# Rocco9999/2048_Q-Learning

Measured on AMD Instinct MI355X. Metric: env_steps_per_sec, higher is better.
Workload: dtype u8

## Files before the change

2048_q-learning_amd/csrc/q2048_core.hpp:

```cpp
#pragma once
#include <stdint.h>
#include <math.h>

#if defined(__HIPCC__)
#define Q_HD __host__ __device__ __forceinline__
#else
#define Q_HD inline
#endif

#include "q2048_luts.inc"

namespace q2048 {

constexpr uint32_t kStreamStep = 0u, kStreamReset = 1u, kStreamOver = 2u;

struct Draws { uint32_t x0, x1, x2, x3; };

#ifndef Q2048_PHILOX_ROUNDS
#define Q2048_PHILOX_ROUNDS 10
#endif
Q_HD Draws philox4x32_10(uint32_t c0, uint32_t c1, uint32_t c2, uint32_t c3, uint32_t k0,
                         uint32_t k1) {
#pragma unroll
  for (int r = 0; r < Q2048_PHILOX_ROUNDS; ++r) {
    const uint64_t p0 = (uint64_t)0xD2511F53u * c0;
    const uint64_t p1 = (uint64_t)0xCD9E8D57u * c2;
    const uint32_t n0 = (uint32_t)(p1 >> 32) ^ c1 ^ k0;
    const uint32_t n2 = (uint32_t)(p0 >> 32) ^ c3 ^ k1;
    c1 = (uint32_t)p1;
    c3 = (uint32_t)p0;
    c0 = n0;
    c2 = n2;
    k0 += 0x9E3779B9u;
    k1 += 0xBB67AE85u;
  }
  return Draws{c0, c1, c2, c3};
}

Q_HD Draws draws(uint64_t seed, uint64_t env_id, uint32_t ctr, uint32_t stream) {
  return philox4x32_10((uint32_t)env_id, (uint32_t)(env_id >> 32), ctr, stream, (uint32_t)seed,
                       (uint32_t)(seed >> 32));
}

Q_HD double draw_uniform(uint32_t x) { return (double)x * (1.0 / 4294967296.0); }
Q_HD int draw_action(uint32_t x) { return (int)(x >> 30); }
Q_HD uint32_t draw_index(uint32_t x, uint32_t n) { return (uint32_t)(((uint64_t)x * n) >> 32); }
Q_HD bool draw_is_four(uint32_t x) { return x >= 3865470567u; }

Q_HD uint32_t nz80(uint32_t x) { return (x + 0x7f7f7f7fu) & 0x80808080u; }
Q_HD uint32_t z80(uint32_t x) { return ~(x + 0x7f7f7f7fu) & 0x80808080u; }
Q_HD uint32_t fill80(uint32_t m) { return (m << 1) - (m >> 7); }
Q_HD uint32_t fill7f(uint32_t m) { return m - (m >> 7); }
Q_HD uint32_t bsel(uint32_t m, uint32_t a, uint32_t b) { return (a & m) | (b & ~m); }

struct Board { uint32_t r0, r1, r2, r3; };

Q_HD bool operator==(const Board& a, const Board& b) {
  return ((a.r0 ^ b.r0) | (a.r1 ^ b.r1) | (a.r2 ^ b.r2) | (a.r3 ^ b.r3)) == 0;
}
Q_HD void clear(Board& b) { b = Board{0u, 0u, 0u, 0u}; }

Q_HD Board transpose(const Board& b) {
  const uint32_t a0 = (b.r0 & 0x00ff00ffu) | ((b.r1 & 0x00ff00ffu) << 8);
  const uint32_t a1 = ((b.r0 >> 8) & 0x00ff00ffu) | (b.r1 & 0xff00ff00u);
  const uint32_t b0 = (b.r2 & 0x00ff00ffu) | ((b.r3 & 0x00ff00ffu) << 8);
  const uint32_t b1 = ((b.r2 >> 8) & 0x00ff00ffu) | (b.r3 & 0xff00ff00u);
  return Board{(a0 & 0xffffu) | (b0 << 16), (a1 & 0xffffu) | (b1 << 16),
               (a0 >> 16) | (b0 & 0xffff0000u), (a1 >> 16) | (b1 & 0xffff0000u)};
}

Q_HD uint32_t pow2_sum(uint32_t v) {
  return (((1u << (v & 0xffu)) & ~1u) + ((1u << ((v >> 8) & 0xffu)) & ~1u)) +
         (((1u << ((v >> 16) & 0xffu)) & ~1u) + ((1u << (v >> 24)) & ~1u));
}

Q_HD uint32_t slide_lines(uint32_t& c0, uint32_t& c1, uint32_t& c2, uint32_t& c3) {
  uint32_t z;
#pragma unroll
  for (int rep = 0; rep < 3; ++rep) {
    z = fill7f(z80(c0));
    c0 = bsel(z, c1, c0); c1 = bsel(z, c2, c1); c2 = bsel(z, c3, c2); c3 &= ~z;
  }
#pragma unroll
  for (int rep = 0; rep < 2; ++rep) {
    z = fill7f(z80(c1));
    c1 = bsel(z, c2, c1); c2 = bsel(z, c3, c2); c3 &= ~z;
  }
  z = fill7f(z80(c2));
  c2 = bsel(z, c3, c2); c3 &= ~z;
  uint32_t e = z80(c0 ^ c1) & nz80(c0);
  uint32_t m = fill7f(e);
  c0 += e >> 7;
  const uint32_t s_a = c0 & m;
  c1 = bsel(m, c2, c1); c2 = bsel(m, c3, c2); c3 &= ~m;
// ... 43 lines not shown
  c = popc(mask & 0x3u);  ge = k >= c; k -= ge ? c : 0u; pos += ge ? 2u : 0u; mask >>= ge ? 2u : 0u;
  c = mask & 1u;          ge = k >= c; pos += ge ? 1u : 0u;
  return pos;
}

Q_HD void put_cell(Board& b, uint32_t pos, uint32_t v) {
  const uint32_t w = v << ((pos & 3u) * 8u), row = pos >> 2;
  b.r0 |= row == 0u ? w : 0u; b.r1 |= row == 1u ? w : 0u;
  b.r2 |= row == 2u ? w : 0u; b.r3 |= row == 3u ? w : 0u;
}

Q_HD void spawn(Board& b, uint32_t draw_pos, uint32_t draw_val) {
  const uint32_t em = empty_mask(b), n = popc(em);
  if (n == 0u) return;
  put_cell(b, kth_set_bit16(em, draw_index(draw_pos, n)), draw_is_four(draw_val) ? 2u : 1u);
}

Q_HD bool game_over(const Board& b) {
  const uint32_t empties = z80(b.r0) | z80(b.r1) | z80(b.r2) | z80(b.r3);
  const uint32_t vert = z80(b.r0 ^ b.r1) | z80(b.r1 ^ b.r2) | z80(b.r2 ^ b.r3);
  const uint32_t horz = (z80(b.r0 ^ (b.r0 >> 8)) | z80(b.r1 ^ (b.r1 >> 8)) |
                         z80(b.r2 ^ (b.r2 >> 8)) | z80(b.r3 ^ (b.r3 >> 8))) & 0x00808080u;
  return (empties | vert | horz) == 0u;
}

Q_HD uint32_t bytemax(uint32_t a, uint32_t b) {
  const uint32_t m = fill7f(((a | 0x80808080u) - b) & 0x80808080u);
  return bsel(m, a, b);
}
Q_HD uint32_t max_log2(const Board& b) {
  uint32_t x = bytemax(bytemax(b.r0, b.r1), bytemax(b.r2, b.r3));
  x = bytemax(x, x >> 16);
  x = bytemax(x, x >> 8);
  return x & 0xffu;
}

struct Aux {
  int32_t score;
  float ep_return;
  uint8_t prev_max;
  uint8_t cons_action;
  uint16_t cons_count;
  uint32_t episode;
};
constexpr uint8_t kNoAction = 0xFFu;
constexpr uint32_t kConsCountSat = 60000u;

Q_HD Aux aux_init() { return Aux{0, 0.0f, 1, kNoAction, 0, 0u}; }

Q_HD double lut_pow12(uint32_t L) { constexpr double t[32] = Q2048_POW12; return t[L & 31u]; }
Q_HD double lut_log2p1(uint32_t L) { constexpr double t[32] = Q2048_LOG2P1; return t[L & 31u]; }
Q_HD double lut_stall(uint32_t k) { constexpr double t[32] = Q2048_STALL; return t[k < 31u ? k : 31u]; }

Q_HD uint64_t f64_bits(double d) { union { double d; uint64_t u; } c; c.d = d; return c.u; }
Q_HD double bits_f64(uint64_t u) { union { double d; uint64_t u; } c; c.u = u; return c.d; }

Q_HD double log2_ge1(double x) {
  constexpr double inv[64] = Q2048_LOG2_INV;
  constexpr double lg[64] = Q2048_LOG2_LG;
  constexpr double a[6] = Q2048_LOG2_COEF;
  const uint64_t u = f64_bits(x);
  const int e = (int)(u >> 52) - 1023;
  const uint32_t j = (uint32_t)(u >> 46) & 63u;
  const double m = bits_f64((u & 0x000FFFFFFFFFFFFFull) | 0x3FF0000000000000ull);
  const double r = fma(m, inv[j], -1.0);
  double p = fma(r, a[5], a[4]);
  p = fma(r, p, a[3]);
  p = fma(r, p, a[2]);
  p = fma(r, p, a[1]);
  p = fma(r, p, a[0]);
  return fma(r, p, (double)e + lg[j]);
}

Q_HD double normalize_reward(double r) {
  const double v = fmin(log2_ge1(fabs(r) + 1.0), 10.0);
  return r >= 0 ? v : -v;
}

Q_HD double calculate_reward(uint32_t score, bool valid, bool over, uint32_t L, uint8_t& prev) {
  L = L < 1u ? 1u : L;
  const double cl = (double)L;
  double bonus = 0.0, r;
  if (L > prev) {
    bonus = (cl - (double)prev) * lut_pow12(L);
    prev = (uint8_t)L;
  }
  if (!valid) {
    if (over) {
      if (L >= 9u && L <= 11u) r = bonus + lut_pow12(L);
      else r = 0.0 - lut_log2p1(L);
    } else {
      r = 0.0 - 0.1 * cl;
    }
  } else {
    r = (double)score;
    if (bonus > 0) r += bonus;
    else r += cl * 0.05;
    if (L >= 9u) r += lut_pow12(L) * 2;
  }
  return normalize_reward(r);
}

struct StepOut {
  float reward;
  double reward64;
  uint32_t score;
  uint8_t done, max_log2, valid;
};

template <class BoardT>
Q_HD bool spawn_then_over(BoardT& b, bool valid, uint32_t x_pos, uint32_t x_val) {
  if (valid) spawn(b, x_pos, x_val);
  return game_over(b);
}

template <class BoardT>
Q_HD StepOut env_step(BoardT& b, Aux& a, int action, uint32_t x_pos, uint32_t x_val) {
  StepOut o;
  uint32_t score;
  const bool valid = move(b, action, score);
  const bool over = spawn_then_over(b, valid, x_pos, x_val);
  const uint32_t mx = max_log2(b);
  a.score += (int32_t)score;
  double r = calculate_reward(score, valid, over, mx, a.prev_max);
  uint32_t cnt = a.cons_count;
  if ((uint8_t)action == a.cons_action) {
    cnt = cnt + 1u < kConsCountSat ? cnt + 1u : kConsCountSat;
  } else {
    a.cons_action = (uint8_t)action;
    cnt = 1u;
  }
  a.cons_count = (uint16_t)cnt;
  bool done = !valid && over;
  if (cnt > 10u) {
    if (cnt > 100u) done = true;
    r += lut_stall(cnt - 10u);
  }
  o.reward64 = r;
  o.reward = (float)r;
  a.ep_return += o.reward;
  o.score = score;
  o.done = done;
  o.max_log2 = (uint8_t)mx;
  o.valid = valid;
  return o;
}

constexpr int kEnvDqn = 1, kEnvResetShaping = 2, kEnvPlayOnly = 4;

template <class BoardT>
Q_HD StepOut env_step_dqn(BoardT& b, Aux& a, int action, uint32_t x_pos, uint32_t x_val,
                          uint32_t y_pos, uint32_t y_val) {
  StepOut o;
  const BoardT pre = b;
  uint32_t score;
  const bool valid = move(b, action, score);
  if (valid) spawn(b, x_pos, x_val);
  bool over = false;
  if (empty_mask(pre) == 0u) {
    over = true;
    for (int act = 0; act < 4 && over; ++act) {
      BoardT t = pre;
      uint32_t s2;
      if (move(t, act, s2)) {
        spawn(t, y_pos, y_val);
        b = t;
        over = false;
      }
    }
    if (over) b = pre;
  }
  const uint32_t mx = max_log2(b);
  a.score += (int32_t)score;
  const double r = (!valid && !over) ? -10.0 : (double)score;
  o.reward64 = r;
  o.reward = (float)r;
  a.ep_return += o.reward;
  o.score = score;
  o.done = over;
  o.max_log2 = (uint8_t)mx;
  o.valid = valid;
  return o;
}

template <int ENV, class BoardT>
Q_HD StepOut env_step_profile(BoardT& b, Aux& a, int action, uint32_t x_pos, uint32_t x_val,
                              uint32_t y_pos, uint32_t y_val) {
  if constexpr ((ENV & kEnvDqn) != 0) return env_step_dqn(b, a, action, x_pos, x_val, y_pos, y_val);
  else return env_step(b, a, action, x_pos, x_val);
}

template <class BoardT>
Q_HD void reset_board(BoardT& b, Aux& a, const Draws& d) {
  clear(b);
  spawn(b, d.x0, d.x1);
  spawn(b, d.x2, d.x3);
  a.score = 0;
  a.ep_return = 0.0f;
}

template <class BoardT>
Q_HD void init_env(BoardT& b, Aux& a, uint64_t seed, uint64_t env_id) {
  a = aux_init();
  reset_board(b, a, draws(seed, env_id, 0u, kStreamReset));
}
template <class BoardT>
Q_HD void begin_episode(BoardT& b, Aux& a, uint64_t seed, uint64_t env_id,
                        bool reset_shaping = false) {
  a.episode += 1u;
  reset_board(b, a, draws(seed, env_id, a.episode, kStreamReset));
  if (reset_shaping) {
    a.prev_max = 1;
    a.cons_action = kNoAction;
    a.cons_count = 0;
  }
}

struct Words4 { uint32_t w0, w1, w2, w3; };
Q_HD uint32_t f32_bits(float f) { union { float f; uint32_t u; } c; c.f = f; return c.u; }
Q_HD float bits_f32(uint32_t u) { union { float f; uint32_t u; } c; c.u = u; return c.f; }
Q_HD Words4 aux_to_words(const Aux& a) {
  return Words4{(uint32_t)a.score, f32_bits(a.ep_return),
                (uint32_t)a.prev_max | ((uint32_t)a.cons_action << 8) | ((uint32_t)a.cons_count << 16),
                a.episode};
}
Q_HD Aux words_to_aux(const Words4& w) {
  return Aux{(int32_t)w.w0, bits_f32(w.w1), (uint8_t)(w.w2 & 0xffu), (uint8_t)((w.w2 >> 8) & 0xffu),
             (uint16_t)(w.w2 >> 16), w.w3};
}

Q_HD uint32_t pack_row(uint32_t x) {
  x &= 0x0f0f0f0fu;
  x = (x | (x >> 4)) & 0x00ff00ffu;
  return (x | (x >> 8)) & 0xffffu;
}
Q_HD uint64_t pack_key(const Board& b, bool& overflow) {
  overflow = ((b.r0 | b.r1 | b.r2 | b.r3) & 0xf0f0f0f0u) != 0u;
  return (uint64_t)(pack_row(b.r0) | (pack_row(b.r1) << 16)) |
         ((uint64_t)(pack_row(b.r2) | (pack_row(b.r3) << 16)) << 32);
}
Q_HD uint32_t unpack_row(uint32_t k) {
  k &= 0xffffu;
  k = (k | (k << 8)) & 0x00ff00ffu;
  return (k | (k << 4)) & 0x0f0f0f0fu;
}
Q_HD Board unpack_key(uint64_t key) {
  return Board{unpack_row((uint32_t)key), unpack_row((uint32_t)(key >> 16)),
               unpack_row((uint32_t)(key >> 32)), unpack_row((uint32_t)(key >> 48))};
}

Q_HD uint64_t mix64(uint64_t h) {
  h *= 0x9E3779B97F4A7C15ull;
  h ^= h >> 29;
  h *= 0xBF58476D1CE4E5B9ull;
  h ^= h >> 32;
  return h;
}
Q_HD uint64_t lane_salt(uint64_t env_id) { return mix64(env_id + 0x2048ull) | 1ull; }

Q_HD uint64_t summary_fp(uint64_t hash) { return ((hash >> 48) & 0xffffull) | 1ull; }
struct SummaryHits { uint32_t ev, empty; };
Q_HD SummaryHits summary_decode(uint64_t word, uint64_t fp, uint32_t off) {
  uint32_t e = 0u, m = 0u;
#pragma unroll
  for (uint32_t r = 0; r < 4u; ++r) {
    const uint64_t f = (word >> (16u * r)) & 0xffffull;
    e |= (uint32_t)(f == 0ull) << r;
    m |= (uint32_t)(f == fp) << r;
  }
  return SummaryHits{(((e | m) | ((e | m) << 4)) >> (off & 3u)) & 15u, e};
}
Q_HD bool summary_pop(SummaryHits& h, uint32_t off, uint32_t& r, bool& absent) {
  if (h.ev == 0u) return false;
  r = (off + (uint32_t)__builtin_ctz(h.ev)) & 3u;
  absent = ((h.empty >> r) & 1u) != 0u;
  h.ev &= h.ev - 1u;
  return true;
}

Q_HD int argmax4(float q0, float q1, float q2, float q3) {
  int b = 0;
  float m = q0;
  if (q1 > m) { m = q1; b = 1; }
  if (q2 > m) { m = q2; b = 2; }
  if (q3 > m) { m = q3; b = 3; }
  return b;
}
Q_HD float max4(float q0, float q1, float q2, float q3) { return fmaxf(fmaxf(q0, q1), fmaxf(q2, q3)); }

Q_HD int eps_greedy(double eps, uint32_t x_eps, uint32_t x_act, float q0, float q1, float q2,
                    float q3, bool& explored) {
  explored = draw_uniform(x_eps) < eps;
  return explored ? draw_action(x_act) : argmax4(q0, q1, q2, q3);
}

#if defined(__clang__)
#define Q2048_NO_CONTRACT _Pragma("clang fp contract(off)")
#else
#define Q2048_NO_CONTRACT
#endif
Q_HD double td_target(float reward, float max_q_next, bool done, double gamma) {
  Q2048_NO_CONTRACT
  const double bootstrap = gamma * (double)max_q_next;
  return (double)reward + bootstrap * (done ? 0.0 : 1.0);
}
Q_HD double td_fold(double q, double target, double lr) {
  Q2048_NO_CONTRACT
  const double step = lr * (target - q);
  return q + step;
}
Q_HD float td_value(float q_sa, float reward, float max_q_next, bool done, double lr,
                    double gamma) {
  return (float)td_fold((double)q_sa, td_target(reward, max_q_next, done, gamma), lr);
}

constexpr uint32_t kRtIdx = 65536u;
Q_HD float rt_sum(float e0, float e1, float e2, float e3) { return (e0 + e1) + (e2 + e3); }
Q_HD float rt_delta(float q_sa, float reward, float max_next, bool done, double lr, double gamma) {
  const double target = (double)reward + (gamma * (double)max_next * (done ? 0.0 : 1.0));
  return (float)((lr * 0.25) * (target - (double)q_sa));
}

}
```

2048_q-learning_amd/csrc/q2048_host.cpp:

```cpp
#include <algorithm>
#include <chrono>
#include <cstddef>
#include <cstdint>
#include <cstdlib>
#include <cstring>
#include <thread>
#include <unordered_map>
#include <vector>

#include "q2048.h"
#include "q2048_core5.hpp"

namespace {
using namespace q2048;
using u64 = unsigned long long;

constexpr uint32_t kMaxProbe = 1u << 14, kRolloutProbe = 1u << 10;
constexpr int kMaxCas = 16;
constexpr int kMaxAwait = 1 << 20;

static_assert(sizeof(q2048_aux) == 16 && sizeof(q2048_slot) == 32 && sizeof(q2048_episode) == 48, "ABI layout");
static_assert(sizeof(Aux) == sizeof(q2048_aux), "core/ABI aux mismatch");

template <int N> struct Geo;
// ... 217 lines not shown
  std::vector<std::thread> th;
  th.reserve((size_t)T);
  for (int t = 0; t < T; ++t) {
    const int64_t lo = B * t / T, hi = B * (t + 1) / T;
    th.emplace_back([=] { f(lo, hi, t); });
  }
  for (auto& x : th) x.join();
  return T;
}

struct Stats {
  uint64_t i[Q2048_NSTAT_I] = {};
  double f[Q2048_NSTAT_F] = {};
  void episode(const Aux& a, uint32_t max_l2) {
    i[Q2048_ST_SCORE] += (uint64_t)(int64_t)a.score;
    i[Q2048_ST_HIST0 + (max_l2 > 22u ? 22u : max_l2)] += 1;
    const double ret = (double)a.ep_return;
    f[Q2048_SF_RETURN] += ret;
    f[Q2048_SF_RETURN_SQ] += ret * ret;
  }
};
void stats_merge(const std::vector<Stats>& parts, int used, int64_t* gi, double* gf) {
  for (int t = 0; t < used; ++t) {
    if (gi != nullptr) for (int k = 0; k < Q2048_NSTAT_I; ++k) gi[k] += (int64_t)parts[(size_t)t].i[k];
    if (gf != nullptr) for (int k = 0; k < Q2048_NSTAT_F; ++k) gf[k] += parts[(size_t)t].f[k];
  }
}

inline bool aligned16(const void* p) { return (reinterpret_cast<uintptr_t>(p) & 15u) == 0; }
inline int check_batch(int64_t B, int n) {
  if (n != 4 && n != 5) return Q2048_ERR_UNSUPPORTED;
  if (B < 0 || B > (int64_t)0x7fffffff * 256) return Q2048_ERR_SIZE;
  return Q2048_OK;
}
inline int check_table(const void* table, int cap_log2) {
  if (table == nullptr) return Q2048_ERR_NULL;
  if (cap_log2 < 4 || cap_log2 > 40) return Q2048_ERR_SIZE;
  if (!aligned16(table)) return Q2048_ERR_ALIGN;
  return Q2048_OK;
}
constexpr uint32_t kAbiFlags = Q2048_FLAG_INDEPENDENT | Q2048_FLAG_SINGLE_ENV | Q2048_FLAG_TD_CAS | Q2048_FLAG_ENV_DQN |
                               Q2048_FLAG_RESET_SHAPING | Q2048_FLAG_PLAY_ONLY | Q2048_FLAG_NO_LEARN |
                               Q2048_FLAG_NO_NEW_ROWS | Q2048_FLAG_LINE_SUMMARY;
inline int check_flags(uint32_t flags, uint32_t refused = 0u) {
  return ((flags & ~kAbiFlags) || (flags & refused)) ? Q2048_ERR_FLAGS : Q2048_OK;
}
inline int env_bits(uint32_t flags) {
  return ((flags & Q2048_FLAG_ENV_DQN) ? kEnvDqn : 0) | ((flags & Q2048_FLAG_RESET_SHAPING) ? kEnvResetShaping : 0);
}
template <class BoardT>
inline StepOut env_step_any(int env, BoardT& b, Aux& a, int act, uint32_t x_pos, uint32_t x_val, uint32_t y_pos, uint32_t y_val) {
  return (env & kEnvDqn) ? env_step_profile<kEnvDqn>(b, a, act, x_pos, x_val, y_pos, y_val)
                         : env_step_profile<0>(b, a, act, x_pos, x_val, y_pos, y_val);
}

template <int N>
void env_init_impl(uint8_t* boards, q2048_aux* aux, int64_t B, uint64_t seed, uint64_t env_id0) {
  parallel_ranges(B, [=](int64_t lo, int64_t hi, int) {
    for (int64_t i = lo; i < hi; ++i) {
      typename Geo<N>::BoardT b;
      Aux a;
      init_env(b, a, seed, env_id0 + (uint64_t)i);
      store_board(boards, i, b);
      st_aux(aux, i, a);
    }
  });
}
template <int N>
void env_reset_impl(uint8_t* boards, q2048_aux* aux, const uint8_t* mask, int64_t B, uint64_t seed, uint64_t env_id0,
                    uint32_t flags) {
  parallel_ranges(B, [=](int64_t lo, int64_t hi, int) {
    for (int64_t i = lo; i < hi; ++i) {
      if (mask != nullptr && mask[i] == 0) continue;
      typename Geo<N>::BoardT b;
      load_board(boards, i, b);
      Aux a = ld_aux(aux, i);
      begin_episode(b, a, seed, env_id0 + (uint64_t)i, (flags & Q2048_FLAG_RESET_SHAPING) != 0);
      store_board(boards, i, b);
      st_aux(aux, i, a);
    }
  });
}
template <int N>
void env_step_impl_n(const uint8_t* boards_in, uint8_t* boards, q2048_aux* aux, const uint8_t* actions, int64_t B,
                     uint64_t seed, uint64_t env_id0, uint32_t ctr, uint32_t flags, float* reward, uint8_t* done,
                     uint8_t* max_l2, int32_t* max_tile, uint32_t* status, const uint32_t* draw_pos,
                     const uint32_t* draw_val, const uint32_t* draw_opos, const uint32_t* draw_oval, int stride) {
  const int env = env_bits(flags);
  parallel_ranges(B, [=](int64_t lo, int64_t hi, int) {
    for (int64_t i = lo; i < hi; ++i) {
      typename Geo<N>::BoardT b;
      load_board(boards_in, i, b);
      const int act = actions[i];
      if (act > 3) {
        status_or(status, Q2048_STATUS_BAD_ACTION);
        reward[i] = 0.f; done[i] = 0; max_l2[i] = 0;
        if (max_tile != nullptr) max_tile[i] = 0;
        if (boards != boards_in) store_board(boards, i, b);
        continue;
      }
      Aux a = ld_aux(aux, i);
      Draws x{0u, 0u, 0u, 0u}, y{0u, 0u, 0u, 0u};
      if (draw_pos != nullptr) {
        x.x2 = draw_pos[i * stride]; x.x3 = draw_val[i * stride];
        if (env & kEnvDqn) { y.x0 = draw_opos[i * stride]; y.x1 = draw_oval[i * stride]; }
      } else {
// ... 93 lines not shown
      const auto key_n = state_key(b_n, salt, status);
      Row rs, rn;
      bool ins_s = false, ins_n = false;
      const int64_t slot = find_or_create(table, mask, key_s, rs, ins_s, create);
      if (slot < 0 && !create) visit_get<N>(cache, i, table, mask, key_s, rs);
      rn = rs;
      const bool same = key_eq(key_n, key_s);
      int64_t slot_n = slot;
      if (!same) slot_n = find_or_create(table, mask, key_n, rn, ins_n, create);
      st.i[Q2048_ST_INSERTS] += (uint64_t)ins_s + (uint64_t)ins_n;
      const float max_next = max4(rn.q0, rn.q1, rn.q2, rn.q3);
      if (slot >= 0) {
        td_update(&table[slot], act, row_get(rs, act), reward[i], max_next, done[i] != 0, lr, gamma, cas, tdc);
      } else {
        st.i[Q2048_ST_DROPS] += 1;
        if (create) status_or(status, Q2048_STATUS_TABLE_FULL);
        else if (same) row_set(rn, act, td_value(row_get(rs, act), reward[i], max_next, done[i] != 0, lr, gamma));
      }
      visit_put<N>(cache, i, table, mask, key_n, rn, !create && slot_n < 0);
    }
    st.i[Q2048_ST_CAS_RETRY] += tdc.retries;
    st.i[Q2048_ST_CAS_FALLBACK] += tdc.fallbacks;
  });
  stats_merge(parts, used, stats_i, nullptr);
}

template <int N>
void q_lookup_impl_n(const q2048_slot* table, u64 mask, const uint8_t* boards, int64_t B, uint64_t env_id0,
                     uint32_t flags, float* q_out, uint8_t* found, uint32_t* status) {
  parallel_ranges(B, [=](int64_t lo, int64_t hi, int) {
    for (int64_t i = lo; i < hi; ++i) {
      typename Geo<N>::BoardT b;
      load_board(boards, i, b);
      const uint64_t id = (flags & Q2048_FLAG_SINGLE_ENV) ? env_id0 : env_id0 + (uint64_t)i;
      const u64 salt = (flags & Q2048_FLAG_INDEPENDENT) ? lane_salt(id) : 0ull;
      Row r;
      const int64_t slot = probe_find(table, mask, state_key(b, salt, status), r, kMaxProbe);
      q_out[4 * i] = r.q0; q_out[4 * i + 1] = r.q1; q_out[4 * i + 2] = r.q2; q_out[4 * i + 3] = r.q3;
      if (found != nullptr) found[i] = slot >= 0;
    }
  });
}

constexpr int kGroup = 16;
template <int N>
void fused_rollout_n(uint8_t* boards, q2048_aux* aux, q2048_slot* table, u64 mask, int64_t B, int steps, double eps,
                     double lr, double gamma, uint64_t seed, uint64_t env_id0, uint32_t ctr0, uint32_t flags,
                     int64_t* stats_i, double* stats_f, uint32_t* status, q2048_episode* log, int64_t log_cap,
                     uint64_t* log_count, void* cache, const uint64_t* side) {
  using BoardT = typename Geo<N>::BoardT;
  using Key = typename Geo<N>::Key;
  struct Lane {
    BoardT b; Aux a; Key key_s, key_n; Row q; int64_t slot_s; u64 salt; uint64_t id; double reward_sum;
    StepOut o; int act; bool explored, same;
  };
  const int env = env_bits(flags);
  const bool play_only = (flags & Q2048_FLAG_PLAY_ONLY) != 0, no_learn = (flags & Q2048_FLAG_NO_LEARN) != 0;
  const bool learns = !play_only && !no_learn, frozen = (flags & Q2048_FLAG_NO_NEW_ROWS) != 0;
  const bool creates = learns && !frozen, cas = (flags & Q2048_FLAG_TD_CAS) != 0;
  const bool summary = N == 5 && learns && frozen && (flags & Q2048_FLAG_LINE_SUMMARY) != 0 && side != nullptr;
  const int T = threads_for(B);
  std::vector<Stats> parts((size_t)T);
  Stats* sp = parts.data();
  const int used = parallel_ranges(B, [=](int64_t lo, int64_t hi, int tid) {
    auto find = [=](const Key& key, Row& row) {
      return summary ? probe_find_summary(table, side, mask, key, row) : probe_find(table, mask, key, row);
    };
    Stats& st = sp[tid];
    TdCounters tdc;
    bool any_drop = false;
    Lane lane[kGroup];
    for (int64_t g0 = lo; g0 < hi; g0 += kGroup) {
      const int n = (int)(hi - g0 < kGroup ? hi - g0 : kGroup);
      for (int l = 0; l < n; ++l) {
        Lane& L = lane[l];
        const int64_t i = g0 + l;
        L.id = env_id0 + (uint64_t)i;
        L.salt = (flags & Q2048_FLAG_INDEPENDENT) ? lane_salt(L.id) : 0ull;
        load_board(boards, i, L.b);
        L.a = ld_aux(aux, i);
        L.key_s = state_key(L.b, L.salt, status);
        L.q = Row{0.f, 0.f, 0.f, 0.f};
        L.slot_s = play_only ? kNoSlot : find(L.key_s, L.q);
        if (frozen && learns && L.slot_s < 0) visit_get<N>(cache, i, table, mask, L.key_s, L.q);
        L.reward_sum = 0.0;
      }
      for (int t = 0; t < steps; ++t) {
        for (int l = 0; l < n; ++l) {
          Lane& L = lane[l];
          const Draws x = draws(seed, L.id, ctr0 + (uint32_t)t, kStreamStep);
          Draws y{0u, 0u, 0u, 0u};
          if (env & kEnvDqn) y = draws(seed, L.id, ctr0 + (uint32_t)t, kStreamOver);
          L.act = eps_greedy(eps, x.x0, x.x1, L.q.q0, L.q.q1, L.q.q2, L.q.q3, L.explored);
          L.o = env_step_any(env, L.b, L.a, L.act, x.x2, x.x3, y.x0, y.x1);
          L.key_n = state_key(L.b, L.salt, status);
          L.same = key_eq(L.key_n, L.key_s);
          if (!L.same && !play_only) __builtin_prefetch(&table[key_hash(L.key_n) & mask], 1, 1);
        }
        for (int l = 0; l < n; ++l) {
          Lane& L = lane[l];
          const StepOut& o = L.o;
          const int act = L.act;
          bool ins_s = false, ins_n = false;
          if (L.slot_s < 0 && L.slot_s != kNoSlot && creates) L.slot_s = probe_insert(table, mask, L.key_s, (u64)~L.slot_s, ins_s);
          Row qn = L.q;
          int64_t slot_n = L.slot_s;
          if (!L.same) {
            if (play_only) { qn = Row{0.f, 0.f, 0.f, 0.f}; slot_n = kNoSlot; }
            else if (creates) slot_n = find_or_create(table, mask, L.key_n, qn, ins_n);
            else slot_n = find(L.key_n, qn);
          }
          const float max_next = max4(qn.q0, qn.q1, qn.q2, qn.q3);
          const bool updated = L.slot_s >= 0;
          float nq = 0.f;
          if (updated) {
            if (no_learn) nq = td_value(row_get(L.q, act), o.reward, max_next, o.done != 0, lr, gamma);
            else nq = td_update(&table[L.slot_s], act, row_get(L.q, act), o.reward, max_next, o.done != 0, lr, gamma, cas, tdc);
          } else if (frozen && learns) {
            nq = td_value(row_get(L.q, act), o.reward, max_next, o.done != 0, lr, gamma);
          }
          st.i[Q2048_ST_VALID] += o.valid != 0;
          st.i[Q2048_ST_EXPLORE] += L.explored;
          st.i[Q2048_ST_INSERTS] += (uint64_t)ins_s + (uint64_t)ins_n;
          if (!updated && learns) { st.i[Q2048_ST_DROPS] += 1; any_drop = any_drop || !frozen; }
          L.reward_sum += (double)o.reward;
          if (o.done) {
            st.i[Q2048_ST_EPISODES] += 1;
            st.episode(L.a, o.max_log2);
            if (log != nullptr) {
              const uint64_t at = __atomic_fetch_add(log_count, (uint64_t)1, __ATOMIC_RELAXED);
              if ((int64_t)at < log_cap) {
                Row ql = L.q;
                if ((updated || (frozen && learns)) && !no_learn) row_set(ql, act, nq);
                q2048_episode rec;
                rec.env_id = L.id; rec.episode = L.a.episode; rec.action = (uint8_t)act;
                rec.max_log2 = o.max_log2; rec.steps_lo = (uint16_t)(ctr0 + (uint32_t)t);
                rec.reward = o.reward; rec.total_return = L.a.ep_return; rec.score = L.a.score;
                rec.q[0] = ql.q0; rec.q[1] = ql.q1; rec.q[2] = ql.q2; rec.q[3] = ql.q3;
                rec.reserved = 0u;
                log[at] = rec;
              }
            }
            begin_episode(L.b, L.a, seed, L.id, (env & kEnvResetShaping) != 0);
            L.key_s = state_key(L.b, L.salt, status);
            L.q = Row{0.f, 0.f, 0.f, 0.f};
            L.slot_s = play_only ? kNoSlot : find(L.key_s, L.q);
          } else if (L.same) {
// ... 675 lines not shown
```

2048_q-learning_amd/csrc/q2048_kernels.hip:

```cpp
#include <hip/hip_runtime.h>
#include <stddef.h>
#include <stdint.h>

#include <cstdio>
#include <cstdlib>
#include <cstring>
#include <ctime>
#include <condition_variable>
#include <deque>
#include <functional>
#include <map>
#include <mutex>
#include <thread>
#include <vector>

#include "q2048.h"
#include "q2048_core5.hpp"

#ifdef Q2048_EXPERIMENTS
#define Q2048_XBITS(flags, shift, mask) (((flags) >> (shift)) & (mask))
#else
#define Q2048_XBITS(flags, shift, mask) 0u
#endif

// ... 848 lines not shown
      Row rn = rs;
      int64_t slot_n = slot;
      Claim claim{0ull, 0ull, false};
      if (!same) {
        slot_n = probe_find(table, mask, key_n, rn, ins_n);
        if constexpr (!frozen) slot_n = claim_issue(table, mask, slot_n, key_n, claim, ins_n);
      }
      const float max_next = max4(rn.q0, rn.q1, rn.q2, rn.q3);
      if (slot >= 0) {
        const float nq = td_update(&table[slot], act, row_get(rs, act), rew, max_next, is_done,
                                   lr, gamma, tdc, td_mode_of(flags));
        if (same) row_set(rn, act, nq);
      } else {
        dropped = true;
        if (!frozen) atomicOr(status, Q2048_STATUS_TABLE_FULL);
        else if (same)
          row_set(rn, act, td_value(row_get(rs, act), rew, max_next, is_done, lr, gamma));
      }
      bool ins_c = false;
      slot_n = claim_resolve(table, mask, key_n, claim, slot_n, ins_c);
      ins_n = ins_n || ins_c;
      if (cache != nullptr) cache_put(cache, i, key_n, cache_tag(table, mask), rn, slot_n, frozen);
    }
    const uint32_t n_ins = wave_count(ins_n) + wave_count(ins_s), n_drop = wave_count(dropped);
    if (tdc.retries) atomicAdd(&bs.i[Q2048_ST_CAS_RETRY], (u64)tdc.retries);
    if (tdc.fallbacks) atomicAdd(&bs.i[Q2048_ST_CAS_FALLBACK], (u64)tdc.fallbacks);
    if (wave_leader()) {
      if (n_ins) atomicAdd(&bs.i[Q2048_ST_INSERTS], (u64)n_ins);
      if (n_drop) atomicAdd(&bs.i[Q2048_ST_DROPS], (u64)n_drop);
    }
  }
  stats_flush(bs, stats_i, nullptr);
}

#ifdef Q2048_FUSED_MIN_WAVES
#define Q2048_FUSED_WAVES(N) Q2048_FUSED_MIN_WAVES
#else
#define Q2048_FUSED_WAVES(N) ((N) == 4 ? 6 : 5)
#endif
constexpr int kModeLearn = 0, kModeCas = 1, kModeEval = 2, kModeFrozen = 4, kModeSummary = 8;
constexpr int kFusedBlockBig = 512, kFusedBlockSmall = kBlock;
constexpr int64_t kFusedBigBatch = 786432;
#ifdef Q2048_EXPERIMENTS
__device__ unsigned long long* g_timeline;
#define Q2048_STAMP(k) do { if (g_timeline != nullptr && threadIdx.x == 0) {                       \
    g_timeline[(size_t)blockIdx.x * 8 + (k)] = wall_clock64();                                     \
    if ((k) == 0) {                                                                                \
      g_timeline[(size_t)blockIdx.x * 8 + 4] = (unsigned)__builtin_amdgcn_s_getreg((31 << 11) | 4);   \
      g_timeline[(size_t)blockIdx.x * 8 + 5] = (unsigned)__builtin_amdgcn_s_getreg((31 << 11) | 20);  \
    } } } while (0)
#else
#define Q2048_STAMP(k) do { } while (0)
#endif
template <int N, int ENV, int MODE, int BLOCK>
__global__ __launch_bounds__(BLOCK, Q2048_FUSED_WAVES(N)) void k_fused_rollout(
    uint8_t* boards, q2048_aux* aux, q2048_slot* table, u64 mask, int64_t B, int steps, double eps,
    double lr, double gamma, uint64_t seed, uint64_t env_id0, uint32_t ctr0, uint32_t flags,
    int64_t* stats_i, double* stats_f, uint32_t* status, q2048_episode* log, int64_t log_cap,
    u64* log_count, void* row_cache, u64* mirror, uint32_t* ticket, const u64* side) {
  RowCache<N>* const cache = static_cast<RowCache<N>*>(row_cache);
  __shared__ BlockStats bs;
  __shared__ Stage<N, BLOCK / 64> st;
  Q2048_STAMP(0);
  stats_clear(bs);
  const int64_t i = (int64_t)blockIdx.x * BLOCK + threadIdx.x;
  auto b = load_board(boards, i, B, st);
  if (i < B) {
    const uint64_t id = env_id0 + (uint64_t)i;
    const u64 salt = (flags & Q2048_FLAG_INDEPENDENT) ? lane_salt(id) : 0ull;
    constexpr bool play_only = (ENV & kEnvPlayOnly) != 0;
    constexpr bool no_learn = MODE == kModeEval;
    constexpr bool frozen = (MODE & kModeFrozen) != 0;
    constexpr bool summary = (MODE & kModeSummary) != 0;
#ifdef Q2048_EXPERIMENTS
    const uint32_t td_mode = no_learn ? (uint32_t)kTdNone : td_mode_of(flags);
    const bool x_noclaim = ((flags >> 12) & 1u) || play_only || no_learn || frozen, x_noprobe = ((flags >> 13) & 1u) || play_only;
    const bool may_defer = td_mode == kTdStorePlain && !((flags >> 14) & 1u);
    const int max_cas = ((flags >> 16) & 0xffu) ? (int)((flags >> 16) & 0xffu) : kMaxCas;
#else
    constexpr uint32_t td_mode = no_learn ? kTdNone : ((MODE & kModeCas) ? kTdCas : kTdStorePlain);
    constexpr bool x_noclaim = play_only || no_learn || frozen, x_noprobe = play_only;
    constexpr bool may_defer = td_mode == kTdStorePlain;
    constexpr int max_cas = kMaxCas;
#endif
    Aux a = ld_aux(aux, i);
    auto key_s = state_key(b, salt, status);
    Row q{0.f, 0.f, 0.f, 0.f};
    bool made0 = false;
    int64_t slot_s = kNoSlot;
    if (!play_only && (cache == nullptr || !cache_get(cache, i, key_s, cache_tag(table, mask), q, slot_s, frozen)))
      slot_s = probe_find_as<summary>(table, side, mask, key_s, q, made0);
    Claim claim{0ull, 0ull, false};
    uint32_t n_valid = 0, n_explore = 0, n_done = 0, n_insert = wave_count(made0), n_drop = 0;
    uint32_t pend = 0;
    TdCounters tdc{0u, 0u};
    double reward_sum = 0.0;

    for (int t = 0; t < steps; ++t) {
      const Draws x = draws(seed, id, ctr0 + (uint32_t)t, kStreamStep);
      Draws y{0u, 0u, 0u, 0u};
      if constexpr ((ENV & kEnvDqn) != 0) y = draws(seed, id, ctr0 + (uint32_t)t, kStreamOver);
      bool explored;
      const int act = eps_greedy(eps, x.x0, x.x1, q.q0, q.q1, q.q2, q.q3, explored);
      const StepOut o = env_step_profile<ENV>(b, a, act, x.x2, x.x3, y.x0, y.x1);
      const auto key_n = state_key(b, salt, status);
      const bool same = key_eq(key_n, key_s);
      bool ins_s = false, ins_n = false;
      slot_s = claim_resolve(table, mask, key_s, claim, slot_s, ins_s);
      if (slot_s < 0 && slot_s != kNoSlot && !x_noclaim)
        slot_s = probe_insert(table, mask, key_s, (u64)~slot_s, ins_s);
      Row qn = q;
      int64_t slot_n = slot_s;
      if (!same) {
        if (x_noprobe) { qn = Row{0.f, 0.f, 0.f, 0.f}; slot_n = ~(int64_t)key_home(key_n, mask); }
        else slot_n = probe_find_as<summary>(table, side, mask, key_n, qn, ins_n);
      }
      const float max_next = max4(qn.q0, qn.q1, qn.q2, qn.q3);
      float nq = 0.f;
      const bool updated = slot_s >= 0;
      if (updated) {
        if (same && !o.done && may_defer) {
          nq = td_value(row_get(q, act), o.reward, max_next, false, lr, gamma);
          pend |= 1u << act;
        } else {
          nq = td_update(&table[slot_s], act, row_get(q, act), o.reward, max_next, o.done != 0, lr,
                         gamma, tdc, td_mode, max_cas);
          pend &= ~(1u << act);
          if (pend) flush_pending(&table[slot_s], q, pend);
        }
      } else if (frozen) {
        nq = td_value(row_get(q, act), o.reward, max_next, o.done != 0, lr, gamma);
      }
      if (o.done) {
        if (!same && slot_n < 0 && slot_n != kNoSlot && !x_noclaim)
          probe_insert(table, mask, key_n, (u64)~slot_n, ins_n);
        episode_stats(bs, a, o.max_log2);
        if (log != nullptr) {
          const u64 at = atomicAdd(log_count, 1ull);
          if ((int64_t)at < log_cap) {
            Row ql = q;
            if ((updated || frozen) && !no_learn) row_set(ql, act, nq);
            q2048_episode rec;
            rec.env_id = id; rec.episode = a.episode; rec.action = (uint8_t)act;
            rec.max_log2 = o.max_log2; rec.steps_lo = (uint16_t)(ctr0 + (uint32_t)t);
            rec.reward = o.reward; rec.total_return = a.ep_return; rec.score = a.score;
            rec.q[0] = ql.q0; rec.q[1] = ql.q1; rec.q[2] = ql.q2; rec.q[3] = ql.q3;
            rec.reserved = 0u;
            log[at] = rec;
          }
        }
        begin_episode(b, a, seed, id, (ENV & kEnvResetShaping) != 0);
        key_s = state_key(b, salt, status);
        bool made = false;
        q = Row{0.f, 0.f, 0.f, 0.f};
        slot_s = play_only ? kNoSlot : probe_find_as<summary>(table, side, mask, key_s, q, made);
        ins_n = ins_n || made;
      } else if (same) {
// ... 2006 lines not shown
```

Before: 22.11 billion.

## Hoist loop-invariant Philox rounds, integer epsilon threshold, and LDS-staged reward LUTs

Precomputes the loop-invariant part of the first two Philox rounds once per environment, so each step only runs the counter-dependent remainder. Replaces the double-precision epsilon comparison with an integer threshold compare on the raw draw. Stages the reward and log2 lookup tables in shared memory per block instead of using per-thread constexpr arrays that may be materialised in scratch or registers. This adds LDS usage and a fill step at kernel start, and it carries a small risk of epsilon-rounding or synchronisation subtleties, since no barrier follows the LDS fill.

Measured after the change: 22.68 billion, median of 6. 2.6% higher.

```diff
diff --git a/2048_q-learning_amd/csrc/q2048_core.hpp b/2048_q-learning_amd/csrc/q2048_core.hpp
--- a/2048_q-learning_amd/csrc/q2048_core.hpp
+++ b/2048_q-learning_amd/csrc/q2048_core.hpp
@@ -19,20 +19,25 @@
 #ifndef Q2048_PHILOX_ROUNDS
 #define Q2048_PHILOX_ROUNDS 10
 #endif
+Q_HD void philox_round(uint32_t& c0, uint32_t& c1, uint32_t& c2, uint32_t& c3, uint32_t k0, uint32_t k1) {
+  const uint64_t p0 = (uint64_t)0xD2511F53u * c0;
+  const uint64_t p1 = (uint64_t)0xCD9E8D57u * c2;
+  const uint32_t n0 = (uint32_t)(p1 >> 32) ^ c1 ^ k0;
+  const uint32_t n2 = (uint32_t)(p0 >> 32) ^ c3 ^ k1;
+  c1 = (uint32_t)p1;
+  c3 = (uint32_t)p0;
+  c0 = n0;
+  c2 = n2;
+}
+constexpr uint32_t kPhiloxW0 = 0x9E3779B9u, kPhiloxW1 = 0xBB67AE85u;
+
 Q_HD Draws philox4x32_10(uint32_t c0, uint32_t c1, uint32_t c2, uint32_t c3, uint32_t k0,
                          uint32_t k1) {
 #pragma unroll
   for (int r = 0; r < Q2048_PHILOX_ROUNDS; ++r) {
-    const uint64_t p0 = (uint64_t)0xD2511F53u * c0;
-    const uint64_t p1 = (uint64_t)0xCD9E8D57u * c2;
-    const uint32_t n0 = (uint32_t)(p1 >> 32) ^ c1 ^ k0;
-    const uint32_t n2 = (uint32_t)(p0 >> 32) ^ c3 ^ k1;
-    c1 = (uint32_t)p1;
-    c3 = (uint32_t)p0;
-    c0 = n0;
-    c2 = n2;
-    k0 += 0x9E3779B9u;
-    k1 += 0xBB67AE85u;
+    philox_round(c0, c1, c2, c3, k0, k1);
+    k0 += kPhiloxW0;
+    k1 += kPhiloxW1;
   }
   return Draws{c0, c1, c2, c3};
 }
@@ -40,6 +45,36 @@
 Q_HD Draws draws(uint64_t seed, uint64_t env_id, uint32_t ctr, uint32_t stream) {
   return philox4x32_10((uint32_t)env_id, (uint32_t)(env_id >> 32), ctr, stream, (uint32_t)seed,
                        (uint32_t)(seed >> 32));
+}
+
+static_assert(Q2048_PHILOX_ROUNDS >= 2, "draws_prepare folds the first two rounds");
+struct DrawPrep {
+  uint32_t a;
+  uint32_t b;
+  uint32_t c;
+  uint32_t d;
+  uint32_t k0, k1;
+};
+Q_HD DrawPrep draws_prepare(uint64_t seed, uint64_t env_id, uint32_t stream) {
+  const uint32_t k0 = (uint32_t)seed, k1 = (uint32_t)(seed >> 32);
+  const uint64_t p0 = (uint64_t)0xD2511F53u * (uint32_t)env_id;
+  const uint32_t n2 = (uint32_t)(p0 >> 32) ^ stream ^ k1;
+  const uint64_t p1 = (uint64_t)0xCD9E8D57u * n2;
+  return DrawPrep{(uint32_t)(env_id >> 32) ^ k0, (uint32_t)(p1 >> 32) ^ (k0 + kPhiloxW0),
+                  (uint32_t)p0 ^ (k1 + kPhiloxW1), (uint32_t)p1, k0 + 2u * kPhiloxW0, k1 + 2u * kPhiloxW1};
+}
+Q_HD Draws draws_at(const DrawPrep& p, uint32_t ctr) {
+  const uint64_t q1 = (uint64_t)0xCD9E8D57u * ctr;
+  const uint64_t q0 = (uint64_t)0xD2511F53u * ((uint32_t)(q1 >> 32) ^ p.a);
+  uint32_t c0 = p.b ^ (uint32_t)q1, c1 = p.d, c2 = (uint32_t)(q0 >> 32) ^ p.c, c3 = (uint32_t)q0;
+  uint32_t k0 = p.k0, k1 = p.k1;
+#pragma unroll
+  for (int r = 2; r < Q2048_PHILOX_ROUNDS; ++r) {
+    philox_round(c0, c1, c2, c3, k0, k1);
+    k0 += kPhiloxW0;
+    k1 += kPhiloxW1;
+  }
+  return Draws{c0, c1, c2, c3};
 }
 
 Q_HD double draw_uniform(uint32_t x) { return (double)x * (1.0 / 4294967296.0); }
@@ -189,43 +224,65 @@
 Q_HD double lut_log2p1(uint32_t L) { constexpr double t[32] = Q2048_LOG2P1; return t[L & 31u]; }
 Q_HD double lut_stall(uint32_t k) { constexpr double t[32] = Q2048_STALL; return t[k < 31u ? k : 31u]; }
 
+
+struct LutImage { double pow12[32], log2p1[32], stall[32], log2_inv[64], log2_lg[64]; };
+#define Q2048_LUT_IMAGE { Q2048_POW12, Q2048_LOG2P1, Q2048_STALL, Q2048_LOG2_INV, Q2048_LOG2_LG }
+constexpr int kLutImageDoubles = (int)(sizeof(LutImage) / sizeof(double));
+struct ConstLuts {
+  Q_HD double pow12(uint32_t L) const { return lut_pow12(L); }
+  Q_HD double log2p1(uint32_t L) const { return lut_log2p1(L); }
+  Q_HD double stall(uint32_t k) const { return lut_stall(k); }
+  Q_HD double log2_inv(uint32_t j) const { constexpr double t[64] = Q2048_LOG2_INV; return t[j & 63u]; }
+  Q_HD double log2_lg(uint32_t j) const { constexpr double t[64] = Q2048_LOG2_LG; return t[j & 63u]; }
+};
+struct ImageLuts {
+  const LutImage* im;
+  Q_HD double pow12(uint32_t L) const { return im->pow12[L & 31u]; }
+  Q_HD double log2p1(uint32_t L) const { return im->log2p1[L & 31u]; }
+  Q_HD double stall(uint32_t k) const { return im->stall[k < 31u ? k : 31u]; }
+  Q_HD double log2_inv(uint32_t j) const { return im->log2_inv[j & 63u]; }
+  Q_HD double log2_lg(uint32_t j) const { return im->log2_lg[j & 63u]; }
+};
+
 Q_HD uint64_t f64_bits(double d) { union { double d; uint64_t u; } c; c.d = d; return c.u; }
 Q_HD double bits_f64(uint64_t u) { union { double d; uint64_t u; } c; c.u = u; return c.d; }
 
-Q_HD double log2_ge1(double x) {
-  constexpr double inv[64] = Q2048_LOG2_INV;
-  constexpr double lg[64] = Q2048_LOG2_LG;
+template <class LutT = ConstLuts>
+Q_HD double log2_ge1(double x, const LutT& lut = LutT()) {
   constexpr double a[6] = Q2048_LOG2_COEF;
   const uint64_t u = f64_bits(x);
   const int e = (int)(u >> 52) - 1023;
   const uint32_t j = (uint32_t)(u >> 46) & 63u;
   const double m = bits_f64((u & 0x000FFFFFFFFFFFFFull) | 0x3FF0000000000000ull);
-  const double r = fma(m, inv[j], -1.0);
+  const double r = fma(m, lut.log2_inv(j), -1.0);
   double p = fma(r, a[5], a[4]);
   p = fma(r, p, a[3]);
   p = fma(r, p, a[2]);
   p = fma(r, p, a[1]);
   p = fma(r, p, a[0]);
-  return fma(r, p, (double)e + lg[j]);
-}
-
-Q_HD double normalize_reward(double r) {
-  const double v = fmin(log2_ge1(fabs(r) + 1.0), 10.0);
+  return fma(r, p, (double)e + lut.log2_lg(j));
+}
+
+template <class LutT = ConstLuts>
+Q_HD double normalize_reward(double r, const LutT& lut = LutT()) {
+  const double v = fmin(log2_ge1(fabs(r) + 1.0, lut), 10.0);
   return r >= 0 ? v : -v;
 }
 
-Q_HD double calculate_reward(uint32_t score, bool valid, bool over, uint32_t L, uint8_t& prev) {
+template <class LutT = ConstLuts>
+Q_HD double calculate_reward(uint32_t score, bool valid, bool over, uint32_t L, uint8_t& prev,
+                             const LutT& lut = LutT()) {
   L = L < 1u ? 1u : L;
   const double cl = (double)L;
   double bonus = 0.0, r;
   if (L > prev) {
-    bonus = (cl - (double)prev) * lut_pow12(L);
+    bonus = (cl - (double)prev) * lut.pow12(L);
     prev = (uint8_t)L;
   }
   if (!valid) {
     if (over) {
-      if (L >= 9u && L <= 11u) r = bonus + lut_pow12(L);
-      else r = 0.0 - lut_log2p1(L);
+      if (L >= 9u && L <= 11u) r = bonus + lut.pow12(L);
+      else r = 0.0 - lut.log2p1(L);
     } else {
       r = 0.0 - 0.1 * cl;
     }
@@ -233,9 +290,9 @@
     r = (double)score;
     if (bonus > 0) r += bonus;
     else r += cl * 0.05;
-    if (L >= 9u) r += lut_pow12(L) * 2;
-  }
-  return normalize_reward(r);
+    if (L >= 9u) r += lut.pow12(L) * 2;
+  }
+  return normalize_reward(r, lut);
 }
 
 struct StepOut {
@@ -251,15 +308,15 @@
   return game_over(b);
 }
 
-template <class BoardT>
-Q_HD StepOut env_step(BoardT& b, Aux& a, int action, uint32_t x_pos, uint32_t x_val) {
+template <class BoardT, class LutT = ConstLuts>
+Q_HD StepOut env_step(BoardT& b, Aux& a, int action, uint32_t x_pos, uint32_t x_val, const LutT& lut = LutT()) {
   StepOut o;
   uint32_t score;
   const bool valid = move(b, action, score);
   const bool over = spawn_then_over(b, valid, x_pos, x_val);
   const uint32_t mx = max_log2(b);
   a.score += (int32_t)score;
-  double r = calculate_reward(score, valid, over, mx, a.prev_max);
+  double r = calculate_reward(score, valid, over, mx, a.prev_max, lut);
   uint32_t cnt = a.cons_count;
   if ((uint8_t)action == a.cons_action) {
     cnt = cnt + 1u < kConsCountSat ? cnt + 1u : kConsCountSat;
@@ -271,7 +328,7 @@
   bool done = !valid && over;
   if (cnt > 10u) {
     if (cnt > 100u) done = true;
-    r += lut_stall(cnt - 10u);
+    r += lut.stall(cnt - 10u);
   }
   o.reward64 = r;
   o.reward = (float)r;
@@ -320,11 +377,11 @@
   return o;
 }
 
-template <int ENV, class BoardT>
+template <int ENV, class BoardT, class LutT = ConstLuts>
 Q_HD StepOut env_step_profile(BoardT& b, Aux& a, int action, uint32_t x_pos, uint32_t x_val,
-                              uint32_t y_pos, uint32_t y_val) {
+                              uint32_t y_pos, uint32_t y_val, const LutT& lut = LutT()) {
   if constexpr ((ENV & kEnvDqn) != 0) return env_step_dqn(b, a, action, x_pos, x_val, y_pos, y_val);
-  else return env_step(b, a, action, x_pos, x_val);
+  else return env_step(b, a, action, x_pos, x_val, lut);
 }
 
 template <class BoardT>
@@ -431,6 +488,20 @@
   return explored ? draw_action(x_act) : argmax4(q0, q1, q2, q3);
 }
 
+Q_HD uint64_t eps_threshold(double eps) {
+  if (!(eps > 0.0)) return 0ull;
+  if (eps >= 1.0) return 1ull << 32;
+  return (uint64_t)ceil(eps * 4294967296.0);
+}
+Q_HD bool draw_below(uint32_t x, uint64_t threshold) {
+  return (threshold >> 32) != 0ull || x < (uint32_t)threshold;
+}
+Q_HD int eps_greedy_at(uint64_t threshold, uint32_t x_eps, uint32_t x_act, float q0, float q1, float q2,
+                       float q3, bool& explored) {
+  explored = draw_below(x_eps, threshold);
+  return explored ? draw_action(x_act) : argmax4(q0, q1, q2, q3);
+}
+
 #if defined(__clang__)
 #define Q2048_NO_CONTRACT _Pragma("clang fp contract(off)")
 #else
diff --git a/2048_q-learning_amd/csrc/q2048_host.cpp b/2048_q-learning_amd/csrc/q2048_host.cpp
--- a/2048_q-learning_amd/csrc/q2048_host.cpp
+++ b/2048_q-learning_amd/csrc/q2048_host.cpp
@@ -293,6 +293,13 @@
 inline StepOut env_step_any(int env, BoardT& b, Aux& a, int act, uint32_t x_pos, uint32_t x_val, uint32_t y_pos, uint32_t y_val) {
   return (env & kEnvDqn) ? env_step_profile<kEnvDqn>(b, a, act, x_pos, x_val, y_pos, y_val)
                          : env_step_profile<0>(b, a, act, x_pos, x_val, y_pos, y_val);
+}
+const LutImage g_lut_image = Q2048_LUT_IMAGE;
+template <class BoardT>
+inline StepOut env_step_any(int env, BoardT& b, Aux& a, int act, uint32_t x_pos, uint32_t x_val, uint32_t y_pos, uint32_t y_val,
+                            const ImageLuts& lut) {
+  return (env & kEnvDqn) ? env_step_profile<kEnvDqn>(b, a, act, x_pos, x_val, y_pos, y_val, lut)
+                         : env_step_profile<0>(b, a, act, x_pos, x_val, y_pos, y_val, lut);
 }
 
 template <int N>
@@ -492,8 +499,10 @@
   using Key = typename Geo<N>::Key;
   struct Lane {
     BoardT b; Aux a; Key key_s, key_n; Row q; int64_t slot_s; u64 salt; uint64_t id; double reward_sum;
-    StepOut o; int act; bool explored, same;
+    StepOut o; int act; bool explored, same; DrawPrep prep;
   };
+  const uint64_t eps_t = eps_threshold(eps);
+  const ImageLuts lut{&g_lut_image};
   const int env = env_bits(flags);
   const bool play_only = (flags & Q2048_FLAG_PLAY_ONLY) != 0, no_learn = (flags & Q2048_FLAG_NO_LEARN) != 0;
   const bool learns = !play_only && !no_learn, frozen = (flags & Q2048_FLAG_NO_NEW_ROWS) != 0;
@@ -524,15 +533,16 @@
         L.slot_s = play_only ? kNoSlot : find(L.key_s, L.q);
         if (frozen && learns && L.slot_s < 0) visit_get<N>(cache, i, table, mask, L.key_s, L.q);
         L.reward_sum = 0.0;
+        L.prep = draws_prepare(seed, L.id, kStreamStep);
       }
       for (int t = 0; t < steps; ++t) {
         for (int l = 0; l < n; ++l) {
           Lane& L = lane[l];
-          const Draws x = draws(seed, L.id, ctr0 + (uint32_t)t, kStreamStep);
+          const Draws x = draws_at(L.prep, ctr0 + (uint32_t)t);
           Draws y{0u, 0u, 0u, 0u};
           if (env & kEnvDqn) y = draws(seed, L.id, ctr0 + (uint32_t)t, kStreamOver);
-          L.act = eps_greedy(eps, x.x0, x.x1, L.q.q0, L.q.q1, L.q.q2, L.q.q3, L.explored);
-          L.o = env_step_any(env, L.b, L.a, L.act, x.x2, x.x3, y.x0, y.x1);
+          L.act = eps_greedy_at(eps_t, x.x0, x.x1, L.q.q0, L.q.q1, L.q.q2, L.q.q3, L.explored);
+          L.o = env_step_any(env, L.b, L.a, L.act, x.x2, x.x3, y.x0, y.x1, lut);
           L.key_n = state_key(L.b, L.salt, status);
           L.same = key_eq(L.key_n, L.key_s);
           if (!L.same && !play_only) __builtin_prefetch(&table[key_hash(L.key_n) & mask], 1, 1);
diff --git a/2048_q-learning_amd/csrc/q2048_kernels.hip b/2048_q-learning_amd/csrc/q2048_kernels.hip
--- a/2048_q-learning_amd/csrc/q2048_kernels.hip
+++ b/2048_q-learning_amd/csrc/q2048_kernels.hip
@@ -924,6 +924,7 @@
 #else
 #define Q2048_STAMP(k) do { } while (0)
 #endif
+__device__ const LutImage g_lut_image = Q2048_LUT_IMAGE;
 template <int N, int ENV, int MODE, int BLOCK>
 __global__ __launch_bounds__(BLOCK, Q2048_FUSED_WAVES(N)) void k_fused_rollout(
     uint8_t* boards, q2048_aux* aux, q2048_slot* table, u64 mask, int64_t B, int steps, double eps,
@@ -933,8 +934,13 @@
   RowCache<N>* const cache = static_cast<RowCache<N>*>(row_cache);
   __shared__ BlockStats bs;
   __shared__ Stage<N, BLOCK / 64> st;
+  __shared__ LutImage lut_lds;
+  static_assert(BLOCK >= kLutImageDoubles, "one double of the image per thread");
   Q2048_STAMP(0);
+  if (threadIdx.x < kLutImageDoubles)
+    reinterpret_cast<double*>(&lut_lds)[threadIdx.x] = reinterpret_cast<const double*>(&g_lut_image)[threadIdx.x];
   stats_clear(bs);
+  const ImageLuts lut{&lut_lds};
   const int64_t i = (int64_t)blockIdx.x * BLOCK + threadIdx.x;
   auto b = load_board(boards, i, B, st);
   if (i < B) {
@@ -967,14 +973,16 @@
     uint32_t pend = 0;
     TdCounters tdc{0u, 0u};
     double reward_sum = 0.0;
+    const DrawPrep prep_x = draws_prepare(seed, id, kStreamStep);
+    const uint64_t eps_t = eps_threshold(eps);
 
     for (int t = 0; t < steps; ++t) {
-      const Draws x = draws(seed, id, ctr0 + (uint32_t)t, kStreamStep);
+      const Draws x = draws_at(prep_x, ctr0 + (uint32_t)t);
       Draws y{0u, 0u, 0u, 0u};
       if constexpr ((ENV & kEnvDqn) != 0) y = draws(seed, id, ctr0 + (uint32_t)t, kStreamOver);
       bool explored;
-      const int act = eps_greedy(eps, x.x0, x.x1, q.q0, q.q1, q.q2, q.q3, explored);
-      const StepOut o = env_step_profile<ENV>(b, a, act, x.x2, x.x3, y.x0, y.x1);
+      const int act = eps_greedy_at(eps_t, x.x0, x.x1, q.q0, q.q1, q.q2, q.q3, explored);
+      const StepOut o = env_step_profile<ENV>(b, a, act, x.x2, x.x3, y.x0, y.x1, lut);
       const auto key_n = state_key(b, salt, status);
       const bool same = key_eq(key_n, key_s);
       bool ins_s = false, ins_n = false;
```
